# mingfeisun/DeepMimic_mujoco

Hardware: AMD Instinct MI355X
Metric: env-steps/sec (higher is better)
Workload: dtype f64

## Files before the change

deepmimic_mujoco_amd/csrc/slot_kernel.h:

```cpp
#pragma once

#include <cstddef>

#include "env_kernel.h"

namespace dm {

constexpr int SLOTS = 4, SW = 16;
#ifndef DM_SLOT_MAXROWS
#define DM_SLOT_MAXROWS 40
#endif
constexpr int SLOT_MAXROWS = DM_SLOT_MAXROWS, SLOT_MAXLIMROWS = 16, SLOT_MAXCON = 13, SLOT_MAXFRAME = 8, SLOT_MAXCAND = 32, SLOT_BOXSLOTS = 3;
constexpr int SLOT_EXTROWS = SLOT_MAXROWS - 2 * SW;
static_assert(SLOT_EXTROWS == 8 || SLOT_EXTROWS == 0, "the partial third row set holds eight rows (or is absent)");
constexpr int PAIR_PASSES = MAXPAIR / SW;
static_assert(MAXPAIR <= 128 && NG <= 16, "a candidate word holds the pair number in 7 bits and both geom numbers in 4 bits each");
constexpr int DOF_PASSES = (NV + SW - 1) / SW, HINGE_PASSES = (NU + SW - 1) / SW, Q_PASSES = (NQ + SW - 1) / SW, ENT_PASSES = (310 + SW - 1) / SW;

#ifndef DM_SLOT_ASSUME
#define DM_SLOT_ASSUME 31
#endif
#define DM_SLOT_LANE_AT(bit, x) (((DM_SLOT_ASSUME) >> (bit)) & 1 ? dmw::launder_slot_lane(x) : dmw::launder(x))

template <class R>
// ... 639 lines not shown
    }
    SlotSolveLTStep<I - 1, NVEC, R>::run(x, qLD, nxt);
  }
};
template <int NVEC, class R> struct SlotSolveLTStep<0, NVEC, R> { static DM_DEV void run(R (*)[NV], const R*, const R*) {} };
template <int NVEC, class R> DM_DEV void slot_solve_LT(R (*x)[NV], const R* qLD) {
  R cur[14];
  dmw::reload_fence();
  load_factor_row<NV - 1>(cur, qLD);
  SlotSolveLTStep<NV - 1, NVEC, R>::run(x, qLD, cur);
}

template <int D, class R>
DM_DEV void slot_load_dof_operands(R* dst, const SlotShared<R>& s) {
  if constexpr (D < NV) {
#pragma unroll
    for (int r = 0; r < 6; r++) dst[r] = s.cdof[D][r];
    dst[6] = s.qvel[D]; dst[7] = s.qws[D];
  }
}
template <int D, int NS, class R>
struct SlotRowStep {
  static DM_DEV void run(R (*y)[NV], RowAcc<R>* ra, const SlotShared<R>& s, const R* cur) {
    R nxt[8];
    dmw::reload_fence();
    slot_load_dof_operands<D + 1>(nxt, s);
    dmw::sched_fence();
#pragma unroll
    for (int k = 0; k < NS; k++) {
      const int pb = (int)(D < 32 ? (ra[k].plus_lo >> D) & 1u : (ra[k].plus_hi >> (D - 32)) & 1u);
      const int mb = (int)(D < 32 ? (ra[k].minus_lo >> D) & 1u : (ra[k].minus_hi >> (D - 32)) & 1u);
      R j = ra[k].w[0] * cur[0] + ra[k].w[1] * cur[1] + ra[k].w[2] * cur[2] + ra[k].w[3] * cur[3] + ra[k].w[4] * cur[4] + ra[k].w[5] * cur[5];
      j = (j + ra[k].w7) * (R)(pb - mb);
      ra[k].vel += j * cur[6]; ra[k].jws += j * cur[7];
      y[k][D] = j;
      dmw::pin_value(ra[k].vel); dmw::pin_value(ra[k].jws);
    }
    SlotRowStep<D + 1, NS, R>::run(y, ra, s, nxt);
  }
};
template <int NS, class R> struct SlotRowStep<NV, NS, R> { static DM_DEV void run(R (*)[NV], RowAcc<R>*, const SlotShared<R>&, const R*) {} };

template <int CC, int NS, class R>
DM_DEV void slot_acol(R (*AR)[16 * NS], const R (*y)[NV]) {
#pragma unroll
  for (int k = 0; k < NS; k++) {
    R acc0 = 0, acc1 = 0;
#pragma unroll
    for (int d = 0; d + 8 <= NV; d += 8) dmw::row_fmac8<CC % 16>(acc0, acc1, &y[CC / 16][d], &y[k][d]);
#pragma unroll
    for (int d = NV / 8 * 8; d < NV; d += 2) { dmw::row_fmac_old<CC % 16>(acc0, y[CC / 16][d], y[k][d]); dmw::row_fmac_old<CC % 16>(acc1, y[CC / 16][d + 1], y[k][d + 1]); }
    AR[k][CC] = acc0 + acc1;
  }
}
template <int C, int NS, class R>
struct SlotACols {
  static DM_DEV void run(R (*AR)[16 * NS], const R (*y)[NV], int nmax) {
    if constexpr (C < 16 * NS) {
      slot_acol<C, NS, R>(AR, y); slot_acol<C + 1, NS, R>(AR, y); slot_acol<C + 2, NS, R>(AR, y); slot_acol<C + 3, NS, R>(AR, y);
      if (C + 4 < nmax) SlotACols<C + 4, NS, R>::run(AR, y, nmax);
    }
  }
};
template <int CC, int NS, class R>
DM_DEV void slot_warm_col(R (*AR)[16 * NS], R* t, const R* f, const R* ndinv) {
#pragma unroll
  for (int k = 0; k < NS; k++) { AR[k][CC] *= ndinv[k]; dmw::row_fmac_old<CC % 16>(t[k], f[CC / 16], AR[k][CC]); }
}
template <int C, int NS, class R>
struct SlotWarm {
  static DM_DEV void run(R (*AR)[16 * NS], R* t, const R* f, const R* ndinv, int nmax) {
    if constexpr (C < 16 * NS) {
      slot_warm_col<C, NS, R>(AR, t, f, ndinv); slot_warm_col<C + 1, NS, R>(AR, t, f, ndinv); slot_warm_col<C + 2, NS, R>(AR, t, f, ndinv); slot_warm_col<C + 3, NS, R>(AR, t, f, ndinv);
      if (C + 4 < nmax) SlotWarm<C + 4, NS, R>::run(AR, t, f, ndinv, nmax);
    }
  }
};
template <int CC, int NS, class R>
DM_DEV void slot_sweep_rows4(const R (*AR)[16 * NS], R* t, R* tsave, const R* nf0, const R* oh) {
  static_assert(CC % 4 == 0, "row groups of four");
  if constexpr (NS == 1) dmw::pgs_rows4<CC % 16>(t[0], tsave[0], nf0[0], &AR[0][CC], &oh[CC % 16]);
  else dmw::pgs_rows4_2<CC % 16>(t[CC / 16], tsave[CC / 16], t[1 - CC / 16], nf0[CC / 16], &AR[CC / 16][CC], &AR[1 - CC / 16][CC], &oh[CC % 16]);
}
template <int C, int NS, class R>
struct SlotSweep {
  static DM_DEV void run(const R (*AR)[16 * NS], R* t, R* tsave, const R* nf0, const R* oh, int nmax) {
    if constexpr (C < 16 * NS) {
      slot_sweep_rows4<C, NS, R>(AR, t, tsave, nf0, oh);
      if (C + 4 < nmax) SlotSweep<C + 4, NS, R>::run(AR, t, tsave, nf0, oh, nmax);
    }
  }
};
template <int CC, class R>
DM_DEV void slot_assemble_row(R* ws, const R (*fy)[NV], R one) {
#pragma unroll
  for (int d = 0; d + 8 <= NV; d += 8) dmw::row_add8<CC % 16>(&ws[d], &fy[CC / 16][d], one);
#pragma unroll
  for (int d = NV / 8 * 8; d < NV; d++) dmw::row_fmac_old<CC % 16>(ws[d], fy[CC / 16][d], one);
}
template <int C, int NS, class R>
struct SlotAssemble {
  static DM_DEV void run(R* ws, const R (*fy)[NV], R one, int nmax) {
    if constexpr (C < 16 * NS) {
      slot_assemble_row<C, R>(ws, fy, one); slot_assemble_row<C + 1, R>(ws, fy, one); slot_assemble_row<C + 2, R>(ws, fy, one); slot_assemble_row<C + 3, R>(ws, fy, one);
      if (C + 4 < nmax) SlotAssemble<C + 4, NS, R>::run(ws, fy, one, nmax);
    }
  }
};

template <class R>
DM_DEV R row_reduce8(const R* p, int sl) {
  const bool b3 = (sl & 8) != 0, b2 = (sl & 4) != 0, b1 = (sl & 2) != 0;
  R q[4], r2[2];
#pragma unroll
  for (int i = 0; i < 4; i++) { const R keep = b3 ? p[4 + i] : p[i], send = b3 ? p[i] : p[4 + i]; q[i] = keep + dmw::perm_row_mirror(send); }
#pragma unroll
  for (int i = 0; i < 2; i++) { const R keep = b2 ? q[2 + i] : q[i], send = b2 ? q[i] : q[2 + i]; r2[i] = keep + dmw::perm_half_mirror(send); }
  const R keep = b1 ? r2[1] : r2[0], send = b1 ? r2[0] : r2[1];
  R v = keep + dmw::perm_xor2(send);
  v += dmw::perm_xor1(v);
  return v;
}
template <int J, class R>
DM_DEV void slot_ext_col(R (*U)[SLOT_EXTROWS], R* B, const R (*y)[NV], const R* y3) {
#pragma unroll
  for (int k = 0; k < 3; k++) {
    const R* mine = k < 2 ? y[k] : y3;
    R acc0 = 0, acc1 = 0;
#pragma unroll
    for (int d = 0; d + 8 <= NV; d += 8) dmw::row_fmac8<2 * J>(acc0, acc1, &y3[d], &mine[d]);
#pragma unroll
    for (int d = NV / 8 * 8; d < NV; d += 2) { dmw::row_fmac_old<2 * J>(acc0, y3[d], mine[d]); dmw::row_fmac_old<2 * J>(acc1, y3[d + 1], mine[d + 1]); }
    if (k < 2) U[k][J] = acc0 + acc1; else B[J] = acc0 + acc1;
  }
}
template <int J, class R>
struct SlotExtCols {
  static DM_DEV void run(R (*U)[SLOT_EXTROWS], R* B, const R (*y)[NV], const R* y3, int next) {
    if constexpr (J < SLOT_EXTROWS) {
      slot_ext_col<J, R>(U, B, y, y3); slot_ext_col<J + 1, R>(U, B, y, y3); slot_ext_col<J + 2, R>(U, B, y, y3); slot_ext_col<J + 3, R>(U, B, y, y3);
      if (J + 4 < next) SlotExtCols<J + 4, R>::run(U, B, y, y3, next);
    }
  }
};
template <int J, class R>
struct SlotExtWarm {
  static DM_DEV void run(R (*U)[SLOT_EXTROWS], R* B, R* t, R f3, const R* ndinv, R ndinv3, int next) {
    if constexpr (J < SLOT_EXTROWS) {
#pragma unroll
      for (int j = J; j < J + 4; j++) { U[0][j] *= ndinv[0]; U[1][j] *= ndinv[1]; B[j] *= ndinv3; }
      dmw::row_fmac_old<2 * J>(t[0], f3, U[0][J]); dmw::row_fmac_old<2 * J>(t[1], f3, U[1][J]);
      dmw::row_fmac_old<2 * J + 2>(t[0], f3, U[0][J + 1]); dmw::row_fmac_old<2 * J + 2>(t[1], f3, U[1][J + 1]);
      dmw::row_fmac_old<2 * J + 4>(t[0], f3, U[0][J + 2]); dmw::row_fmac_old<2 * J + 4>(t[1], f3, U[1][J + 2]);
      dmw::row_fmac_old<2 * J + 6>(t[0], f3, U[0][J + 3]); dmw::row_fmac_old<2 * J + 6>(t[1], f3, U[1][J + 3]);
      if (J + 4 < next) SlotExtWarm<J + 4, R>::run(U, B, t, f3, ndinv, ndinv3, next);
    }
  }
};
template <class R>
DM_DEV R slot_ext_residual(const R (*U)[SLOT_EXTROWS], const R* B, const R* f, const R* diag, R f3, R tb3, R ndinv3, int sl) {
  const R g0 = -(diag[0] * f[0]), g1 = -(diag[1] * f[1]);
  R p[SLOT_EXTROWS > 0 ? SLOT_EXTROWS : 1];
#pragma unroll
  for (int j = 0; j < SLOT_EXTROWS; j++) p[j] = U[0][j] * g0 + U[1][j] * g1;
  R t3 = tb3 + ndinv3 * row_reduce8(p, sl);
  dmw::dpp_settle();
  dmw::row_fmac_old<0>(t3, f3, B[0]); dmw::row_fmac_old<2>(t3, f3, B[1]); dmw::row_fmac_old<4>(t3, f3, B[2]); dmw::row_fmac_old<6>(t3, f3, B[3]);
  dmw::row_fmac_old<8>(t3, f3, B[4]); dmw::row_fmac_old<10>(t3, f3, B[5]); dmw::row_fmac_old<12>(t3, f3, B[6]); dmw::row_fmac_old<14>(t3, f3, B[7]);
  return t3;
}
template <int J, class R>
struct SlotExtSweep {
  static DM_DEV void run(const R (*U)[SLOT_EXTROWS], const R* B, R& t3, R& tsave3, R* t, R nf03, const R* oh, int next) {
    if constexpr (J < SLOT_EXTROWS) {
      dmw::pgs_row3<2 * J>(t3, tsave3, t[0], t[1], nf03, B[J], U[0][J], U[1][J], oh[2 * J]);
// ... 194 lines not shown
  R AR[NF][NC];
#pragma unroll
  for (int k = 0; k < NF; k++)
#pragma unroll
    for (int c = 0; c < NC; c++) { AR[k][c] = 0; dmw::pin_value(AR[k][c]); }
  dmw::dpp_settle();
  SlotACols<0, NF, R>::run(AR, y, nmax);
  R diag[NF];
#pragma unroll
  for (int k = 0; k < NF; k++) {
    R dg = 1;
#pragma unroll
    for (int c = 0; c < 16; c++) { if (sl == c) { AR[k][16 * k + c] += active[k] ? Rr[k] : R(0); dg = AR[k][16 * k + c]; } }
    diag[k] = active[k] ? dg : R(1);
  }
  SLOT_STAMP(10)
  typedef decltype(dmw::park(R(0))) ParkedR;
  ParkedR ypark[NF == 2 ? NF : 1][NF == 2 ? NV : 1];
  if constexpr (NF == 2) {
    if constexpr (!EXT) {
      if (sl == 0) {
#pragma unroll
        for (int d = 0; d < NV; d++) s.tau[d] = y[NF][d];
      }
    }
#pragma unroll
    for (int k = 0; k < NF; k++)
#pragma unroll
      for (int d = 0; d < NV; d++) ypark[k][d] = dmw::park(y[k][d]);
#pragma unroll
    for (int k = 0; k < NF; k++)
#pragma unroll
      for (int c = 0; c < NC; c++) dmw::pin_value(AR[k][c]);
    if constexpr (EXT) {
#pragma unroll
      for (int j = 0; j < NX; j++) { dmw::pin_value(U[0][j]); dmw::pin_value(U[1][j]); dmw::pin_value(B3[j]); }
    }
  }
  R ndinv[NF], tb[NF], t[NF];
#pragma unroll
  for (int k = 0; k < NF; k++) { ndinv[k] = active[k] ? R(-1) / diag[k] : R(0); dmw::pin_value(ndinv[k]); tb[k] = bb[k] * ndinv[k]; t[k] = tb[k]; }
  SlotWarm<0, NF, R>::run(AR, t, f, ndinv, nmax);
  R ndinv3 = 0, tb3 = 0;
  if constexpr (EXT) {
    ndinv3 = active3 ? R(-1) / diag3 : R(0); dmw::pin_value(ndinv3);
    tb3 = bb3 * ndinv3;
    dmw::dpp_settle();
    SlotExtWarm<0, R>::run(U, B3, t, f3, ndinv, ndinv3, nmax - 2 * SW);
  }
  {
    R c = 0;
#pragma unroll
    for (int k = 0; k < NF; k++) { const R res = -t[k] * diag[k]; c += active[k] ? f[k] * (R(0.5) * (res - bb[k]) + bb[k]) : R(0); }
    if constexpr (EXT) {
      const R t3 = slot_ext_residual(U, B3, f, diag, f3, tb3, ndinv3, sl);
      const R res = -t3 * diag3;
      c += active3 ? f3 * (R(0.5) * (res - bb3) + bb3) : R(0);
    }
    const R cost = dmw::sum16(c);
    if (cost > 0) {
#pragma unroll
      for (int k = 0; k < NF; k++) { f[k] = 0; t[k] = tb[k]; }
      f3 = 0;
    }
  }
  SLOT_STAMP(11)
  const int maxiter = dmw::uniform(M.iterations);
  R pgs_scale = M.pgs_scale, pgs_tol = M.tolerance, pgs_detect = M.pgs_detect;
  dmw::pin_value(pgs_scale); dmw::pin_value(pgs_tol); dmw::pin_value(pgs_detect);
  int iter = 0;
  bool frozen = nefc == 0 || maxiter <= 0, anybad = false;
  if (frozen) {
#pragma unroll
    for (int k = 0; k < NF; k++) t[k] = 0;
  }
  R oh[16];
#pragma unroll
  for (int i = 0; i < 16; i++) { oh[i] = sl == i ? R(1) : R(0); dmw::pin_value(oh[i]); }
  R nf[NF], nf3 = -f3;
#pragma unroll
  for (int k = 0; k < NF; k++) nf[k] = -f[k];
  R pgs_ntol = -pgs_tol;
  dmw::pin_value(pgs_ntol);
  auto sweep = [&](R& chg, bool& bad) {
    const int nm = dmw::launder_uniform(nmax);
    R tsave[NF];
#pragma unroll
    for (int k = 0; k < NF; k++) tsave[k] = 0;
    SlotSweep<0, NF, R>::run(AR, t, tsave, nf, oh, nm);
    bad = false;
#pragma unroll
    for (int k = 0; k < NF; k++) {
      const R delta = dmw::max_raw(nf[k], tsave[k]);
      const R change = (delta * diag[k]) * (R(0.5) * delta - tsave[k]);
      chg = k == 0 ? change : chg + change;
      nf[k] -= delta; bad = bad || (change > pgs_detect);
    }
    if constexpr (EXT) {
      R fnow[NF];
#pragma unroll
      for (int k = 0; k < NF; k++) fnow[k] = -nf[k];
      const R f3now = -nf3;
      R t3 = slot_ext_residual(U, B3, fnow, diag, f3now, tb3, ndinv3, sl);
      t3 = frozen ? R(0) : t3;
      R tsave3 = 0;
      SlotExtSweep<0, R>::run(U, B3, t3, tsave3, t, nf3, oh, nm - 2 * SW);
      const R delta = dmw::max_raw(nf3, tsave3);
      const R change = (delta * diag3) * (R(0.5) * delta - tsave3);
      nf3 -= delta; chg += change; bad = bad || (change > pgs_detect);
    }
  };
  if (dmw::ballot(!frozen) != 0ull) {
    R chg; bool bad;
    sweep(chg, bad);
    if (!frozen) { iter = 1; anybad = bad; }
    bool more = true;
    while (more) {
      R nfprev[NF], nfprev3 = nf3;
#pragma unroll
      for (int k = 0; k < NF; k++) nfprev[k] = nf[k];
      const R schg = dmw::sum16(chg) * pgs_scale;
      R chg2; bool bad2;
      sweep(chg2, bad2);
      const bool act = !frozen;
      const bool conv = (int)act & ((int)(schg > pgs_ntol) | (int)(iter >= maxiter));
#pragma unroll
      for (int k = 0; k < NF; k++) {
        nf[k] = conv ? nfprev[k] : nf[k];
        t[k] = conv ? R(0) : t[k];
      }
      if constexpr (EXT) nf3 = conv ? nfprev3 : nf3;
      const bool go = (int)act & (int)!conv;
      iter += go ? 1 : 0;
      anybad = (int)anybad | ((int)go & (int)bad2);
      frozen = (int)frozen | (int)conv;
      chg = chg2;
      more = dmw::ballot(!frozen) != 0ull;
      if (PROF) prof[6] += 1;
    }
  }
#pragma unroll
  for (int k = 0; k < NF; k++) f[k] = -nf[k];
  f3 = -nf3;
  if (PROF && NS >= 2) { prof[22] += dmw::clk() - pt0; }
  if (PROF && NS == 3) { prof[27] += dmw::clk() - pt0; }
  SLOT_STAMP(12)
  if (PROF) { prof[14] += nmax; prof[15] += 1; }
  if (dmw::row_ballot(anybad, lane) != 0u) ovf |= 16 | 64;
  if (dbg) {
#pragma unroll
    for (int k = 0; k < NF; k++) if (active[k]) {
      double* o = dbg->out + (34 * 34 + 34 * 3 + 42 + 3) + (sl + 16 * k) * (34 + 6) + 34;
      o[0] = (double)pos[k]; o[1] = (double)margin[k]; o[2] = (double)Rr[k]; o[3] = (double)aref[k]; o[4] = (double)bb[k]; o[5] = (double)f[k];
    }
  }
  R fy3[EXT ? NV : 1];
  if constexpr (EXT) {
    const R* y3lds = &s.qd.o.qacc[0];
    const R f3a = active3 ? f3 : R(0);
#pragma unroll
    for (int d = 0; d < NV; d++) { fy3[d] = ((sl & 1) == 0 ? y3lds[d * SLOT_EXTROWS + (sl >> 1)] : R(0)) * f3a; dmw::pin_value(fy3[d]); }
  }
  if constexpr (NF == 2) {
    dmw::sync();
#pragma unroll
    for (int d = 0; d < NV; d++) y[NF][d] = s.tau[d];
  }
#pragma unroll
  for (int k = 0; k < NF; k++) {
    const R fk = active[k] ? f[k] : R(0);
#pragma unroll
    for (int d = 0; d < NV; d++) { if constexpr (NF == 2) y[k][d] = dmw::unpark(ypark[k][d]); y[k][d] *= fk; dmw::pin_value(y[k][d]); }
  }
  R ws[NV];
#pragma unroll
  for (int d = 0; d < NV; d++) { ws[d] = 0; dmw::pin_value(ws[d]); }
  R one = 1;
  dmw::pin_value(one);
  dmw::dpp_settle();
  SlotAssemble<0, NF, R>::run(ws, y, one, nmax);
  if constexpr (EXT) SlotExtAssemble<0, R>::run(ws, fy3, one, nmax - 2 * SW);
#pragma unroll
  for (int d = 0; d < NV; d++) ws[d] = (ws[d] + y[NF][d]) * s.dsq[d];
  solve_L(ws, s.r2.qLD);
  if (sl == 0) {
#pragma unroll
    for (int d = 0; d < NV; d++) s.qd.o.qacc[d] = ws[d];
    s.solver_iter = iter;
  }
  dmw::sync();
  SLOT_STAMP(13)
  if (PROF && NS >= 2) prof[24] += dmw::clk() - pt_enter;
  if (PROF && NS == 3) prof[26] += dmw::clk() - pt_enter;
#undef SLOT_STAMP
}

#if !defined(DM_WAVE_TESTBENCH)
template <class R, int MAXR>
static __device__ __noinline__ int slot_rows_call(const DevModel<R>* M, SlotShared<R>* s, int sl, int lane, int* ovf) {
  int o = *ovf;
  const int n = slot_rows<R, false, MAXR>(*dmw::in_constant(M), *dmw::in_lds(s), sl, lane, o, (long long*)0);
  *ovf = o;
  return n;
}
#endif

template <class R>
DM_DEV void slot_smooth_solve(SlotShared<R>& s, int sl, const DebugOut* dbg) {
  R x[1][NV];
#pragma unroll
  for (int d = 0; d < NV; d++) x[0][d] = s.tau[d];
  slot_solve_LT<1>(x, s.r2.qLD);
#pragma unroll
  for (int d = 0; d < NV; d++) { x[0][d] *= s.dsq[d]; dmw::pin_value(x[0][d]); }
#pragma unroll
  for (int d = 0; d < NV; d++) x[0][d] = (R(0) + x[0][d]) * s.dsq[d];
  solve_L(x[0], s.r2.qLD);
  if (sl == 0) {
#pragma unroll
    for (int d = 0; d < NV; d++) { s.qd.o.qacc[d] = x[0][d]; if (dbg) dbg->out[34 * 34 + 34 + d] = (double)x[0][d]; }
    s.solver_iter = 0;
  }
// ... 57 lines not shown
```

deepmimic_mujoco_amd/csrc/wave.h:

```cpp
#pragma once

#if defined(DM_WAVE_TESTBENCH)
#include "wave_testbench.h"
#else
#include <hip/hip_runtime.h>

#define DM_DEV __device__ __forceinline__
#define DM_DEV_NOINLINE __device__ __noinline__
#ifndef DM_NO_STATIC_CALLS
#define DM_STATIC_CALLS 1
#define DM_DEV_CALL64 static __device__ __noinline__
#else
#define DM_DEV_CALL64 __device__ __noinline__
#endif
#define DM_CONSTANT __device__ constexpr

namespace dmw {
DM_DEV int lane() { return (int)(threadIdx.x & 63u); }
DM_DEV void sync() { __builtin_amdgcn_fence(__ATOMIC_SEQ_CST, "wavefront"); __builtin_amdgcn_wave_barrier(); }
DM_DEV void sync_mem() { __syncthreads(); }
DM_DEV unsigned long long ballot(bool p) { return __ballot(p); }
DM_DEV int shfl_i(int v, int src) { return __shfl(v, src, 64); }
DM_DEV double shfl(double v, int src) { return __shfl(v, src, 64); }
DM_DEV float shfl(float v, int src) { return __shfl(v, src, 64); }
DM_DEV double shfl_xor(double v, int m) { return __shfl_xor(v, m, 64); }
DM_DEV float shfl_xor(float v, int m) { return __shfl_xor(v, m, 64); }
DM_DEV int shfl_xor_i(int v, int m) { return __shfl_xor(v, m, 64); }
DM_DEV int shfl_up_i(int v, int d) { return __shfl_up(v, d, 64); }
DM_DEV double bcast(double v, int src) {
  int lo = __double2loint(v), hi = __double2hiint(v);
  lo = __builtin_amdgcn_readlane(lo, src);
  hi = __builtin_amdgcn_readlane(hi, src);
  return __hiloint2double(hi, lo);
}
DM_DEV float bcast(float v, int src) { return __int_as_float(__builtin_amdgcn_readlane(__float_as_int(v), src)); }
DM_DEV int bcast_i(int v, int src) { return __builtin_amdgcn_readlane(v, src); }
template <int CTRL>
DM_DEV double dpp_f64(double v) {
  int lo = __double2loint(v), hi = __double2hiint(v);
  lo = __builtin_amdgcn_update_dpp(0, lo, CTRL, 0xf, 0xf, true);
  hi = __builtin_amdgcn_update_dpp(0, hi, CTRL, 0xf, 0xf, true);
  return __hiloint2double(hi, lo);
}
template <int CTRL>
DM_DEV float dpp_f32(float v) { return __int_as_float(__builtin_amdgcn_update_dpp(0, __float_as_int(v), CTRL, 0xf, 0xf, true)); }
DM_DEV float perm_xor1(float v) { return dpp_f32<0xB1>(v); }
DM_DEV float perm_xor2(float v) { return dpp_f32<0x4E>(v); }
DM_DEV float perm_half_mirror(float v) { return dpp_f32<0x141>(v); }
DM_DEV float perm_row_mirror(float v) { return dpp_f32<0x140>(v); }
DM_DEV double perm_xor1(double v) { return dpp_f64<0xB1>(v); }
DM_DEV double perm_xor2(double v) { return dpp_f64<0x4E>(v); }
DM_DEV double perm_half_mirror(double v) { return dpp_f64<0x141>(v); }
DM_DEV double perm_row_mirror(double v) { return dpp_f64<0x140>(v); }
DM_DEV int uniform(int v) { return __builtin_amdgcn_readfirstlane(v); }
DM_DEV bool uniform(bool v) { return __builtin_amdgcn_readfirstlane((int)v) != 0; }
DM_DEV double rcp_fast(double x) {
  double r = __builtin_amdgcn_rcp(x);
  double e = __builtin_fma(-x, r, 1.0); r = __builtin_fma(e, r, r);
  e = __builtin_fma(-x, r, 1.0); r = __builtin_fma(e, r, r);
  return r;
}
DM_DEV float rcp_fast(float x) { return 1.0f / x; }
DM_DEV void mfma_16x16x4(double a, double b, double (&d)[4]) {
  typedef double v4d __attribute__((ext_vector_type(4)));
  v4d c = {d[0], d[1], d[2], d[3]};
  c = __builtin_amdgcn_mfma_f64_16x16x4f64(a, b, c, 0, 0, 0);
  d[0] = c[0]; d[1] = c[1]; d[2] = c[2]; d[3] = c[3];
}
DM_DEV void mfma_16x16x4(float a, float b, float (&d)[4]) {
  typedef float v4f __attribute__((ext_vector_type(4)));
  v4f c = {d[0], d[1], d[2], d[3]};
  c = __builtin_amdgcn_mfma_f32_16x16x4f32(a, b, c, 0, 0, 0);
  d[0] = c[0]; d[1] = c[1]; d[2] = c[2]; d[3] = c[3];
}
DM_DEV int mfma_row(int lane_id, int v, double) { return (lane_id >> 4) + 4 * v; }
DM_DEV int mfma_row(int lane_id, int v, float) { return 4 * (lane_id >> 4) + v; }
DM_DEV double max_raw(double a, double b) { double r; asm("v_max_f64 %0, %1, %2" : "=v"(r) : "v"(a), "v"(b)); return r; }
DM_DEV float max_raw(float a, float b) { float r; asm("v_max_f32 %0, %1, %2" : "=v"(r) : "v"(a), "v"(b)); return r; }
DM_DEV long long clk() { return (long long)__builtin_readcyclecounter(); }
DM_DEV void sched_fence() { __builtin_amdgcn_sched_barrier(0); }
DM_DEV int pin_zero() { int z = 0; asm volatile("" : "+s"(z)); return z; }
DM_DEV void pin_value(double& v) { asm volatile("" : "+v"(v)); }
DM_DEV void pin_value(float& v) { asm volatile("" : "+v"(v)); }
DM_DEV int launder(int v) { asm volatile("" : "+v"(v)); return v; }
DM_DEV int launder_slot_lane(int v) { asm volatile("" : "+v"(v)); __builtin_assume(v >= 0 && v < 16); return v; }
DM_DEV unsigned long long launder(unsigned long long v) { asm volatile("" : "+v"(v)); return v; }
DM_DEV int launder_uniform(int v) { asm volatile("" : "+s"(v)); return v; }
template <class T> DM_DEV T* uniform_ptr(T* p) {
  const unsigned long long v = (unsigned long long)p;
  const unsigned lo = __builtin_amdgcn_readfirstlane((unsigned)v), hi = __builtin_amdgcn_readfirstlane((unsigned)(v >> 32));
  return (T*)(((unsigned long long)hi << 32) | lo);
}
template <class T> DM_DEV T* in_lds(T* p) {
#if defined(__HIP_DEVICE_COMPILE__)
  __builtin_assume(__builtin_amdgcn_is_shared((const void*)p));
#endif
  return p;
}
template <class T> DM_DEV T* in_global(T* p) {
  __attribute__((address_space(1))) T* g = (__attribute__((address_space(1))) T*)uniform_ptr(p);
  asm volatile("" : "+s"(g));
  return (T*)g;
}
template <class T> DM_DEV const T* in_constant(const T* p) {
// ... 10 lines not shown
  x = __builtin_amdgcn_update_dpp(0ll, x, 0x150 + I, 0xf, 0xf, true);
  return __longlong_as_double(x);
}
template <int I> DM_DEV float row_bcast(float v) { return __int_as_float(__builtin_amdgcn_update_dpp(0, __float_as_int(v), 0x150 + I, 0xf, 0xf, true)); }
template <int I> DM_DEV int row_bcast_i(int v) { return __builtin_amdgcn_update_dpp(0, v, 0x150 + I, 0xf, 0xf, true); }
template <int I> DM_DEV void row_fmac(double& acc, double x, double y) {
  asm volatile("s_nop 1\n\tv_fmac_f64_dpp %0, %1, %2 row_newbcast:%3 row_mask:0xf bank_mask:0xf" : "+v"(acc) : "v"(x), "v"(y), "n"(I));
}
template <int I> DM_DEV void row_fmac(float& acc, float x, float y) { acc += row_bcast<I>(x) * y; }
template <int I> DM_DEV void row_fmac_old(double& acc, double x, double y) {
  asm volatile("s_nop 1\n\tv_fmac_f64_dpp %0, %1, %2 row_newbcast:%3 row_mask:0xf bank_mask:0xf" : "+v"(acc) : "v"(x), "v"(y), "n"(I));
}
template <int I> DM_DEV void row_fmac_old(float& acc, float x, float y) { acc += row_bcast<I>(x) * y; }
#define DM_FMAC_DPP(acc, x, y) "v_fmac_f64_dpp " acc ", " x ", " y " row_newbcast:%18 row_mask:0xf bank_mask:0xf\n\t"
template <int I> DM_DEV void row_fmac8(double& acc0, double& acc1, const double* x, const double* y) {
  asm volatile("s_nop 1\n\t" DM_FMAC_DPP("%0", "%2", "%10") DM_FMAC_DPP("%1", "%3", "%11") DM_FMAC_DPP("%0", "%4", "%12") DM_FMAC_DPP("%1", "%5", "%13")
               DM_FMAC_DPP("%0", "%6", "%14") DM_FMAC_DPP("%1", "%7", "%15") DM_FMAC_DPP("%0", "%8", "%16") DM_FMAC_DPP("%1", "%9", "%17")
               : "+v"(acc0), "+v"(acc1)
               : "v"(x[0]), "v"(x[1]), "v"(x[2]), "v"(x[3]), "v"(x[4]), "v"(x[5]), "v"(x[6]), "v"(x[7]),
                 "v"(y[0]), "v"(y[1]), "v"(y[2]), "v"(y[3]), "v"(y[4]), "v"(y[5]), "v"(y[6]), "v"(y[7]), "n"(I));
}
#undef DM_FMAC_DPP
#define DM_FMAC_DPP(acc, x) "v_fmac_f64_dpp " acc ", " x ", %16 row_newbcast:%17 row_mask:0xf bank_mask:0xf\n\t"
template <int I> DM_DEV void row_add8(double* a, const double* x, double one) {
  asm volatile("s_nop 1\n\t" DM_FMAC_DPP("%0", "%8") DM_FMAC_DPP("%1", "%9") DM_FMAC_DPP("%2", "%10") DM_FMAC_DPP("%3", "%11")
               DM_FMAC_DPP("%4", "%12") DM_FMAC_DPP("%5", "%13") DM_FMAC_DPP("%6", "%14") DM_FMAC_DPP("%7", "%15")
               : "+v"(a[0]), "+v"(a[1]), "+v"(a[2]), "+v"(a[3]), "+v"(a[4]), "+v"(a[5]), "+v"(a[6]), "+v"(a[7])
               : "v"(x[0]), "v"(x[1]), "v"(x[2]), "v"(x[3]), "v"(x[4]), "v"(x[5]), "v"(x[6]), "v"(x[7]), "v"(one), "n"(I));
}
#undef DM_FMAC_DPP
template <int I> DM_DEV void row_fmac8(float& acc0, float& acc1, const float* x, const float* y) { for (int k = 0; k < 8; k++) { if (k & 1) acc1 += row_bcast<I>(x[k]) * y[k]; else acc0 += row_bcast<I>(x[k]) * y[k]; } }
template <int I> DM_DEV void row_add8(float* a, const float* x, float one) { for (int k = 0; k < 8; k++) a[k] += row_bcast<I>(x[k]) * one; }
template <int I> DM_DEV void pgs_row(double& t, double& tsave, double nf0, double a, double onehot) {
  double delta;
  asm volatile("v_max_f64 %0, %3, %1\n\tv_fma_f64 %2, %5, %1, %2\n\ts_nop 0\n\tv_fmac_f64_dpp %1, %0, %4 row_newbcast:%6 row_mask:0xf bank_mask:0xf"
               : "=&v"(delta), "+v"(t), "+v"(tsave) : "v"(nf0), "v"(a), "v"(onehot), "n"(I));
}
template <int I> DM_DEV void pgs_row2(double& t_own, double& tsave_own, double& t_other, double nf0, double a_own, double a_other, double onehot) {
  double delta;
  asm volatile("v_max_f64 %0, %4, %1\n\tv_fma_f64 %2, %7, %1, %2\n\ts_nop 0\n\tv_fmac_f64_dpp %1, %0, %5 row_newbcast:%8 row_mask:0xf bank_mask:0xf\n\t"
               "v_fmac_f64_dpp %3, %0, %6 row_newbcast:%8 row_mask:0xf bank_mask:0xf"
               : "=&v"(delta), "+v"(t_own), "+v"(tsave_own), "+v"(t_other) : "v"(nf0), "v"(a_own), "v"(a_other), "v"(onehot), "n"(I));
}
template <int I> DM_DEV void pgs_row3(double& t3, double& tsave3, double& t0, double& t1, double nf0, double b, double u0, double u1, double onehot) {
  double delta;
  asm volatile("v_max_f64 %0, %5, %1\n\tv_fma_f64 %2, %9, %1, %2\n\ts_nop 0\n\tv_fmac_f64_dpp %1, %0, %6 row_newbcast:%10 row_mask:0xf bank_mask:0xf\n\t"
               "v_fmac_f64_dpp %3, %0, %7 row_newbcast:%10 row_mask:0xf bank_mask:0xf\n\tv_fmac_f64_dpp %4, %0, %8 row_newbcast:%10 row_mask:0xf bank_mask:0xf"
               : "=&v"(delta), "+v"(t3), "+v"(tsave3), "+v"(t0), "+v"(t1) : "v"(nf0), "v"(b), "v"(u0), "v"(u1), "v"(onehot), "n"(I));
}
template <int I> DM_DEV void pgs_row3(float& t3, float& tsave3, float& t0, float& t1, float nf0, float b, float u0, float u1, float onehot) {
  const float d = max_raw(nf0, t3); tsave3 += onehot * t3; const float bc = row_bcast<I>(d); t3 += bc * b; t0 += bc * u0; t1 += bc * u1;
}
#define DM_PGS1(D, A, OH, I) "v_max_f64 " D ", %3, %0\n\tv_fma_f64 %1, " OH ", %0, %1\n\ts_nop 0\n\tv_fmac_f64_dpp %0, " D ", " A " row_newbcast:" I " row_mask:0xf bank_mask:0xf\n\t"
template <int I0> DM_DEV void pgs_rows4(double& t, double& tsave, double nf0, const double* a, const double* oh) {
  double d;
  asm volatile(DM_PGS1("%2", "%4", "%8", "%12") DM_PGS1("%2", "%5", "%9", "%13") DM_PGS1("%2", "%6", "%10", "%14") DM_PGS1("%2", "%7", "%11", "%15")
               : "+v"(t), "+v"(tsave), "=&v"(d)
               : "v"(nf0), "v"(a[0]), "v"(a[1]), "v"(a[2]), "v"(a[3]), "v"(oh[0]), "v"(oh[1]), "v"(oh[2]), "v"(oh[3]), "n"(I0), "n"(I0 + 1), "n"(I0 + 2), "n"(I0 + 3));
}
#undef DM_PGS1
template <int I0> DM_DEV void pgs_rows4_2(double& t_own, double& tsave_own, double& t_other, double nf0, const double* a_own, const double* a_other, const double* oh) {
  double d0, d1;
  asm volatile(
      "v_max_f64 %3, %5, %0\n\tv_fma_f64 %1, %14, %0, %1\n\ts_nop 0\n\tv_fmac_f64_dpp %0, %3, %6 row_newbcast:%18 row_mask:0xf bank_mask:0xf\n\t"
      "v_max_f64 %4, %5, %0\n\tv_fma_f64 %1, %15, %0, %1\n\tv_fmac_f64_dpp %2, %3, %10 row_newbcast:%18 row_mask:0xf bank_mask:0xf\n\tv_fmac_f64_dpp %0, %4, %7 row_newbcast:%19 row_mask:0xf bank_mask:0xf\n\t"
      "v_max_f64 %3, %5, %0\n\tv_fma_f64 %1, %16, %0, %1\n\tv_fmac_f64_dpp %2, %4, %11 row_newbcast:%19 row_mask:0xf bank_mask:0xf\n\tv_fmac_f64_dpp %0, %3, %8 row_newbcast:%20 row_mask:0xf bank_mask:0xf\n\t"
      "v_max_f64 %4, %5, %0\n\tv_fma_f64 %1, %17, %0, %1\n\tv_fmac_f64_dpp %2, %3, %12 row_newbcast:%20 row_mask:0xf bank_mask:0xf\n\tv_fmac_f64_dpp %0, %4, %9 row_newbcast:%21 row_mask:0xf bank_mask:0xf\n\t"
      "s_nop 0\n\tv_fmac_f64_dpp %2, %4, %13 row_newbcast:%21 row_mask:0xf bank_mask:0xf"
      : "+v"(t_own), "+v"(tsave_own), "+v"(t_other), "=&v"(d0), "=&v"(d1)
      : "v"(nf0), "v"(a_own[0]), "v"(a_own[1]), "v"(a_own[2]), "v"(a_own[3]), "v"(a_other[0]), "v"(a_other[1]), "v"(a_other[2]), "v"(a_other[3]),
        "v"(oh[0]), "v"(oh[1]), "v"(oh[2]), "v"(oh[3]), "n"(I0), "n"(I0 + 1), "n"(I0 + 2), "n"(I0 + 3));
}
template <int I> DM_DEV void pgs_row(float& t, float& tsave, float nf0, float a, float onehot) { const float d = max_raw(nf0, t); tsave += onehot * t; t += row_bcast<I>(d) * a; }
template <int I> DM_DEV void pgs_row2(float& t_own, float& tsave_own, float& t_other, float nf0, float a_own, float a_other, float onehot) {
  const float d = max_raw(nf0, t_own); tsave_own += onehot * t_own; const float b = row_bcast<I>(d); t_own += b * a_own; t_other += b * a_other;
}
template <int I0> DM_DEV void pgs_rows4(float& t, float& tsave, float nf0, const float* a, const float* oh) {
  pgs_row<I0>(t, tsave, nf0, a[0], oh[0]); pgs_row<I0 + 1>(t, tsave, nf0, a[1], oh[1]); pgs_row<I0 + 2>(t, tsave, nf0, a[2], oh[2]); pgs_row<I0 + 3>(t, tsave, nf0, a[3], oh[3]);
}
template <int I0> DM_DEV void pgs_rows4_2(float& t_own, float& tsave_own, float& t_other, float nf0, const float* a_own, const float* a_other, const float* oh) {
  pgs_row2<I0>(t_own, tsave_own, t_other, nf0, a_own[0], a_other[0], oh[0]); pgs_row2<I0 + 1>(t_own, tsave_own, t_other, nf0, a_own[1], a_other[1], oh[1]);
  pgs_row2<I0 + 2>(t_own, tsave_own, t_other, nf0, a_own[2], a_other[2], oh[2]); pgs_row2<I0 + 3>(t_own, tsave_own, t_other, nf0, a_own[3], a_other[3], oh[3]);
}
DM_DEV void dpp_settle() { asm volatile("s_nop 4"); }
struct Parked { int lo, hi; };
DM_DEV Parked park(double v) {
  Parked p;
  asm volatile("v_accvgpr_write_b32 %0, %2\n\tv_accvgpr_write_b32 %1, %3" : "=a"(p.lo), "=a"(p.hi) : "v"(__double2loint(v)), "v"(__double2hiint(v)));
  return p;
}
DM_DEV double unpark(const Parked& p) {
  int lo, hi;
  asm volatile("v_accvgpr_read_b32 %0, %2\n\tv_accvgpr_read_b32 %1, %3" : "=v"(lo), "=v"(hi) : "a"(p.lo), "a"(p.hi));
  return __hiloint2double(hi, lo);
}
struct ParkedF { int x; };
DM_DEV ParkedF park(float v) { ParkedF p; asm volatile("v_accvgpr_write_b32 %0, %1" : "=a"(p.x) : "v"(__float_as_int(v))); return p; }
DM_DEV float unpark(const ParkedF& p) { int x; asm volatile("v_accvgpr_read_b32 %0, %1" : "=v"(x) : "a"(p.x)); return __int_as_float(x); }
DM_DEV int global_counter_next(int* p) { return atomicAdd(p, 1); }
DM_DEV unsigned row_ballot(bool p, int lane_id) { return (unsigned)((__ballot(p) >> (lane_id & 48)) & 0xffffull); }
}
#endif

namespace dmw {
DM_DEV double sum8(double v) { v += perm_xor1(v); v += perm_xor2(v); v += perm_half_mirror(v); return v; }
DM_DEV double sum16(double v) { v = sum8(v); v += perm_row_mirror(v); return v; }
DM_DEV double wave_sum(double v) {
  v = sum16(v);
  return ((bcast(v, 0) + bcast(v, 16)) + bcast(v, 32)) + bcast(v, 48);
}
#if !defined(DM_WAVE_TESTBENCH)
DM_DEV float sum8(float v) { v += perm_xor1(v); v += perm_xor2(v); v += perm_half_mirror(v); return v; }
DM_DEV float sum16(float v) { v = sum8(v); v += perm_row_mirror(v); return v; }
DM_DEV float wave_sum(float v) {
  v = sum16(v);
  return ((bcast(v, 0) + bcast(v, 16)) + bcast(v, 32)) + bcast(v, 48);
}
#endif
DM_DEV int wave_exclusive_scan(int v, int lane_id, int* total) {
  const unsigned long long below = (1ull << lane_id) - 1ull;
  int pre = 0, tot = 0;
#pragma unroll
  for (int b = 0; b < 5; b++) {
    const unsigned long long m = ballot(((v >> b) & 1) != 0);
    pre += __builtin_popcountll(m & below) << b;
    tot += __builtin_popcountll(m) << b;
  }
  *total = tot;
  return pre;
}
}
```

Measured before the change: 20.71 million.

## Overlap PGS convergence reduction with the next sweep's row updates

Interleaves the 16-lane cost-change reduction (DPP stages) into the inline-asm row updates of the following PGS sweep, so the reduction no longer sits serially between sweeps. Loop control is restructured around a trip counter and a cheaper ballot builtin, and the cost change is computed with explicit FMA and non-contracted ops to keep rounding identical. The asm hardcodes v250-v253, which constrains register allocation and could cause spills. It also adds coupling between sweep length and reduction stage count.

New measurement: 20.70 million. No clear change (-0.0%).

```diff
diff --git a/deepmimic_mujoco_amd/csrc/slot_kernel.h b/deepmimic_mujoco_amd/csrc/slot_kernel.h
--- a/deepmimic_mujoco_amd/csrc/slot_kernel.h
+++ b/deepmimic_mujoco_amd/csrc/slot_kernel.h
@@ -745,15 +745,33 @@
   if constexpr (NS == 1) dmw::pgs_rows4<CC % 16>(t[0], tsave[0], nf0[0], &AR[0][CC], &oh[CC % 16]);
   else dmw::pgs_rows4_2<CC % 16>(t[CC / 16], tsave[CC / 16], t[1 - CC / 16], nf0[CC / 16], &AR[CC / 16][CC], &AR[1 - CC / 16][CC], &oh[CC % 16]);
 }
-template <int C, int NS, class R>
+template <int CC, int NS, class R>
+DM_DEV void slot_sweep_rows4_red(const R (*AR)[16 * NS], R* t, R* tsave, const R* nf0, const R* oh, R& red) {
+  static_assert(CC % 4 == 0 && CC < (NS == 1 ? 8 : 16), "row groups of four; four stages");
+  if constexpr (NS == 1) dmw::pgs_rows4_red2<CC, CC / 2>(t[0], tsave[0], nf0[0], &AR[0][CC], &oh[CC], red);
+  else dmw::pgs_rows4_2_red<CC, CC / 4>(t[0], tsave[0], t[1], nf0[0], &AR[0][CC], &AR[1][CC], &oh[CC], red);
+}
+template <int C, int NS, bool RED, class R>
 struct SlotSweep {
-  static DM_DEV void run(const R (*AR)[16 * NS], R* t, R* tsave, const R* nf0, const R* oh, int nmax) {
+  static DM_DEV void run(const R (*AR)[16 * NS], R* t, R* tsave, const R* nf0, const R* oh, int nmax, R& red, R scale) {
     if constexpr (C < 16 * NS) {
-      slot_sweep_rows4<C, NS, R>(AR, t, tsave, nf0, oh);
-      if (C + 4 < nmax) SlotSweep<C + 4, NS, R>::run(AR, t, tsave, nf0, oh, nmax);
+      if constexpr (RED && C < (NS == 1 ? 8 : 16)) slot_sweep_rows4_red<C, NS, R>(AR, t, tsave, nf0, oh, red);
+      else {
+        if constexpr (RED && C == 16) red = dmw::mul_rn(red, scale);
+        slot_sweep_rows4<C, NS, R>(AR, t, tsave, nf0, oh);
+      }
+      if constexpr (C + 4 < 16 * NS) { if (C + 4 < nmax) SlotSweep<C + 4, NS, RED, R>::run(AR, t, tsave, nf0, oh, nmax, red, scale); }
     }
   }
 };
+template <int NS, bool RED, class R>
+DM_DEV void slot_sweep(const R (*AR)[16 * NS], R* t, R* tsave, const R* nf0, const R* oh, int nmax, R& red, R scale) {
+  SlotSweep<0, NS, RED, R>::run(AR, t, tsave, nf0, oh, nmax, red, scale);
+  if constexpr (RED && NS == 1) {
+    if (nmax <= 4) { dmw::dpp_settle(); red = dmw::sum16_stage<3>(dmw::sum16_stage<2>(red)); }
+    red = dmw::mul_rn(red, scale);
+  }
+}
 template <int CC, class R>
 DM_DEV void slot_assemble_row(R* ws, const R (*fy)[NV], R one) {
 #pragma unroll
@@ -1114,19 +1132,23 @@
   for (int k = 0; k < NF; k++) nf[k] = -f[k];
   R pgs_ntol = -pgs_tol;
   dmw::pin_value(pgs_ntol);
-  auto sweep = [&](R& chg, bool& bad) {
+  auto sweep = [&](auto redtag, R& red, R& chg, bool& bad) {
+    constexpr bool RED = decltype(redtag)::value;
     const int nm = dmw::launder_uniform(nmax);
     R tsave[NF];
 #pragma unroll
     for (int k = 0; k < NF; k++) tsave[k] = 0;
-    SlotSweep<0, NF, R>::run(AR, t, tsave, nf, oh, nm);
+    slot_sweep<NF, RED, R>(AR, t, tsave, nf, oh, nm, red, pgs_scale);
     bad = false;
+    static_assert(NF <= 2, "the cost change below is written for one or two row sets");
+    R p0 = 0, q0 = 0;
 #pragma unroll
     for (int k = 0; k < NF; k++) {
       const R delta = dmw::max_raw(nf[k], tsave[k]);
-      const R change = (delta * diag[k]) * (R(0.5) * delta - tsave[k]);
-      chg = k == 0 ? change : chg + change;
-      nf[k] -= delta; bad = bad || (change > pgs_detect);
+      const R p = dmw::mul_rn(delta, diag[k]), q = dmw::mul_sub(R(0.5), delta, tsave[k]);
+      const R change = dmw::mul_rn(p, q);
+      if (k == 0) { chg = change; p0 = p; q0 = q; } else chg = dmw::mul_add(p0, q0, change);
+      nf[k] = dmw::sub_rn(nf[k], delta); bad = bad || (change > pgs_detect);
     }
     if constexpr (EXT) {
       R fnow[NF];
@@ -1143,33 +1165,37 @@
     }
   };
   if (dmw::ballot(!frozen) != 0ull) {
-    R chg; bool bad;
-    sweep(chg, bad);
-    if (!frozen) { iter = 1; anybad = bad; }
+    R chg, none = 0; bool bad;
+    sweep(std::false_type(), none, chg, bad);
+    if (!frozen) anybad = bad;
+    int trip = 1;
+    bool act = !frozen;
+    iter = act ? 0 : -1;
     bool more = true;
     while (more) {
       R nfprev[NF], nfprev3 = nf3;
 #pragma unroll
       for (int k = 0; k < NF; k++) nfprev[k] = nf[k];
-      const R schg = dmw::sum16(chg) * pgs_scale;
+      R schg = chg;
       R chg2; bool bad2;
-      sweep(chg2, bad2);
-      const bool act = !frozen;
-      const bool conv = (int)act & ((int)(schg > pgs_ntol) | (int)(iter >= maxiter));
+      sweep(std::true_type(), schg, chg2, bad2);
+      const bool capped = trip >= maxiter;
+      const bool conv = (int)act & ((int)(schg > pgs_ntol) | (int)capped);
 #pragma unroll
       for (int k = 0; k < NF; k++) {
         nf[k] = conv ? nfprev[k] : nf[k];
         t[k] = conv ? R(0) : t[k];
       }
-      if constexpr (EXT) nf3 = conv ? nfprev3 : nf3;
-      const bool go = (int)act & (int)!conv;
-      iter += go ? 1 : 0;
-      anybad = (int)anybad | ((int)go & (int)bad2);
-      frozen = (int)frozen | (int)conv;
+      if constexpr (EXT) { nf3 = conv ? nfprev3 : nf3; frozen = (int)frozen | (int)conv; }
+      iter = conv ? trip : iter;
+      act = iter == 0;
+      anybad = (int)anybad | ((int)act & (int)bad2);
       chg = chg2;
-      more = dmw::ballot(!frozen) != 0ull;
+      trip++;
+      more = dmw::lane_mask(act) != 0ull;
       if (PROF) prof[6] += 1;
     }
+    iter = iter < 0 ? 0 : iter;
   }
 #pragma unroll
   for (int k = 0; k < NF; k++) f[k] = -nf[k];
diff --git a/deepmimic_mujoco_amd/csrc/wave.h b/deepmimic_mujoco_amd/csrc/wave.h
--- a/deepmimic_mujoco_amd/csrc/wave.h
+++ b/deepmimic_mujoco_amd/csrc/wave.h
@@ -2,6 +2,19 @@
 
 #if defined(DM_WAVE_TESTBENCH)
 #include "wave_testbench.h"
+namespace dmw {
+inline unsigned long long lane_mask(bool pr) { return ballot(pr); }
+template <int S> inline double sum16_stage(double v) {
+  static_assert(S >= 0 && S < 4, "sum16 has four stages");
+  if constexpr (S == 0) return v + perm_xor1(v); else if constexpr (S == 1) return v + perm_xor2(v); else if constexpr (S == 2) return v + perm_half_mirror(v); else return v + perm_row_mirror(v);
+}
+template <int I0, int S, class T> inline void pgs_rows4_red2(T& t, T& tsave, T nf0, const T* a, const T* oh, T& acc) { pgs_rows4<I0>(t, tsave, nf0, a, oh); acc = sum16_stage<S + 1>(sum16_stage<S>(acc)); }
+template <int I0, int S, class T> inline void pgs_rows4_2_red(T& t_own, T& tsave_own, T& t_other, T nf0, const T* a_own, const T* a_other, const T* oh, T& acc) {
+  pgs_rows4_2<I0>(t_own, tsave_own, t_other, nf0, a_own, a_other, oh); acc = sum16_stage<S>(acc);
+}
+template <class T> inline T mul_sub(T a, T b, T c) { return a * b - c; }
+template <class T> inline T mul_add(T a, T b, T c) { return a * b + c; }
+}
 #else
 #include <hip/hip_runtime.h>
 
@@ -20,6 +33,7 @@
 DM_DEV void sync() { __builtin_amdgcn_fence(__ATOMIC_SEQ_CST, "wavefront"); __builtin_amdgcn_wave_barrier(); }
 DM_DEV void sync_mem() { __syncthreads(); }
 DM_DEV unsigned long long ballot(bool p) { return __ballot(p); }
+DM_DEV unsigned long long lane_mask(bool p) { return __builtin_amdgcn_ballot_w64(p); }
 DM_DEV int shfl_i(int v, int src) { return __shfl(v, src, 64); }
 DM_DEV double shfl(double v, int src) { return __shfl(v, src, 64); }
 DM_DEV float shfl(float v, int src) { return __shfl(v, src, 64); }
@@ -196,6 +210,60 @@
   pgs_row2<I0>(t_own, tsave_own, t_other, nf0, a_own[0], a_other[0], oh[0]); pgs_row2<I0 + 1>(t_own, tsave_own, t_other, nf0, a_own[1], a_other[1], oh[1]);
   pgs_row2<I0 + 2>(t_own, tsave_own, t_other, nf0, a_own[2], a_other[2], oh[2]); pgs_row2<I0 + 3>(t_own, tsave_own, t_other, nf0, a_own[3], a_other[3], oh[3]);
 }
+template <int S> DM_DEV double sum16_stage(double v) {
+  static_assert(S >= 0 && S < 4, "sum16 has four stages");
+  if constexpr (S == 0) return v + perm_xor1(v); else if constexpr (S == 1) return v + perm_xor2(v); else if constexpr (S == 2) return v + perm_half_mirror(v); else return v + perm_row_mirror(v);
+}
+template <int S> DM_DEV float sum16_stage(float v) {
+  static_assert(S >= 0 && S < 4, "sum16 has four stages");
+  if constexpr (S == 0) return v + perm_xor1(v); else if constexpr (S == 1) return v + perm_xor2(v); else if constexpr (S == 2) return v + perm_half_mirror(v); else return v + perm_row_mirror(v);
+}
+#define DM_RIDE_LO(CTRL) "v_mov_b32_dpp v252, v250 " CTRL " row_mask:0xf bank_mask:0xf bound_ctrl:1"
+#define DM_RIDE_HI(CTRL) "v_mov_b32_dpp v253, v251 " CTRL " row_mask:0xf bank_mask:0xf bound_ctrl:1"
+#define DM_RIDE_ADD "v_add_f64 v[250:251], v[250:251], v[252:253]"
+#define DM_PGS1R(A, OH, I, SLOT) "v_max_f64 %[d], %[nf0], %[t]\n\tv_fma_f64 %[ts], %[" OH "], %[t], %[ts]\n\t" SLOT "\n\tv_fmac_f64_dpp %[t], %[d], %[" A "] row_newbcast:%[" I "] row_mask:0xf bank_mask:0xf\n\t"
+#define DM_PGS_ROWS4_RED2(CA, CB)                                                                                                                                \
+  asm volatile(DM_PGS1R("a0", "oh0", "i0", DM_RIDE_LO(CA)) DM_PGS1R("a1", "oh1", "i1", DM_RIDE_HI(CA)) DM_PGS1R("a2", "oh2", "i2", DM_RIDE_ADD)                   \
+               DM_PGS1R("a3", "oh3", "i3", DM_RIDE_LO(CB) "\n\t" DM_RIDE_HI(CB)) DM_RIDE_ADD                                                                      \
+               : [t] "+v"(t), [ts] "+v"(tsave), [d] "=&v"(d), "+{v[250:251]}"(acc), "=&{v[252:253]}"(tmp)                                                         \
+               : [nf0] "v"(nf0), [a0] "v"(a[0]), [a1] "v"(a[1]), [a2] "v"(a[2]), [a3] "v"(a[3]), [oh0] "v"(oh[0]), [oh1] "v"(oh[1]), [oh2] "v"(oh[2]), [oh3] "v"(oh[3]), \
+                 [i0] "n"(I0), [i1] "n"(I0 + 1), [i2] "n"(I0 + 2), [i3] "n"(I0 + 3))
+template <int I0, int S> DM_DEV void pgs_rows4_red2(double& t, double& tsave, double nf0, const double* a, const double* oh, double& acc) {
+  static_assert(S == 0 || S == 2, "stages 0, 1 or stages 2, 3");
+  double d, tmp;
+  if constexpr (S == 0) DM_PGS_ROWS4_RED2("quad_perm:[1,0,3,2]", "quad_perm:[2,3,0,1]"); else DM_PGS_ROWS4_RED2("row_half_mirror", "row_mirror");
+}
+#undef DM_PGS_ROWS4_RED2
+#undef DM_PGS1R
+#define DM_PGS_ROWS4_2_RED(CTRL)                                                                                                                                 \
+  asm volatile(                                                                                                                                                  \
+      "v_max_f64 %[d0], %[nf0], %[t]\n\tv_fma_f64 %[ts], %[oh0], %[t], %[ts]\n\t" DM_RIDE_LO(CTRL) "\n\tv_fmac_f64_dpp %[t], %[d0], %[a0] row_newbcast:%[i0] row_mask:0xf bank_mask:0xf\n\t" \
+      "v_max_f64 %[d1], %[nf0], %[t]\n\tv_fma_f64 %[ts], %[oh1], %[t], %[ts]\n\t" DM_RIDE_HI(CTRL) "\n\tv_fmac_f64_dpp %[u], %[d0], %[b0] row_newbcast:%[i0] row_mask:0xf bank_mask:0xf\n\tv_fmac_f64_dpp %[t], %[d1], %[a1] row_newbcast:%[i1] row_mask:0xf bank_mask:0xf\n\t" \
+      "v_max_f64 %[d0], %[nf0], %[t]\n\tv_fma_f64 %[ts], %[oh2], %[t], %[ts]\n\tv_fmac_f64_dpp %[u], %[d1], %[b1] row_newbcast:%[i1] row_mask:0xf bank_mask:0xf\n\tv_fmac_f64_dpp %[t], %[d0], %[a2] row_newbcast:%[i2] row_mask:0xf bank_mask:0xf\n\t" \
+      "v_max_f64 %[d1], %[nf0], %[t]\n\tv_fma_f64 %[ts], %[oh3], %[t], %[ts]\n\tv_fmac_f64_dpp %[u], %[d0], %[b2] row_newbcast:%[i2] row_mask:0xf bank_mask:0xf\n\tv_fmac_f64_dpp %[t], %[d1], %[a3] row_newbcast:%[i3] row_mask:0xf bank_mask:0xf\n\t" \
+      DM_RIDE_ADD "\n\tv_fmac_f64_dpp %[u], %[d1], %[b3] row_newbcast:%[i3] row_mask:0xf bank_mask:0xf"                                                           \
+      : [t] "+v"(t_own), [ts] "+v"(tsave_own), [u] "+v"(t_other), [d0] "=&v"(d0), [d1] "=&v"(d1), "+{v[250:251]}"(acc), "=&{v[252:253]}"(tmp)                     \
+      : [nf0] "v"(nf0), [a0] "v"(a_own[0]), [a1] "v"(a_own[1]), [a2] "v"(a_own[2]), [a3] "v"(a_own[3]), [b0] "v"(a_other[0]), [b1] "v"(a_other[1]),              \
+        [b2] "v"(a_other[2]), [b3] "v"(a_other[3]), [oh0] "v"(oh[0]), [oh1] "v"(oh[1]), [oh2] "v"(oh[2]), [oh3] "v"(oh[3]),                                      \
+        [i0] "n"(I0), [i1] "n"(I0 + 1), [i2] "n"(I0 + 2), [i3] "n"(I0 + 3))
+template <int I0, int S> DM_DEV void pgs_rows4_2_red(double& t_own, double& tsave_own, double& t_other, double nf0, const double* a_own, const double* a_other, const double* oh, double& acc) {
+  static_assert(S >= 0 && S < 4, "sum16 has four stages");
+  double d0, d1, tmp;
+  if constexpr (S == 0) DM_PGS_ROWS4_2_RED("quad_perm:[1,0,3,2]"); else if constexpr (S == 1) DM_PGS_ROWS4_2_RED("quad_perm:[2,3,0,1]");
+  else if constexpr (S == 2) DM_PGS_ROWS4_2_RED("row_half_mirror"); else DM_PGS_ROWS4_2_RED("row_mirror");
+}
+#undef DM_PGS_ROWS4_2_RED
+#undef DM_RIDE_LO
+#undef DM_RIDE_HI
+#undef DM_RIDE_ADD
+template <int I0, int S> DM_DEV void pgs_rows4_red2(float& t, float& tsave, float nf0, const float* a, const float* oh, float& acc) { pgs_rows4<I0>(t, tsave, nf0, a, oh); acc = sum16_stage<S + 1>(sum16_stage<S>(acc)); }
+template <int I0, int S> DM_DEV void pgs_rows4_2_red(float& t_own, float& tsave_own, float& t_other, float nf0, const float* a_own, const float* a_other, const float* oh, float& acc) {
+  pgs_rows4_2<I0>(t_own, tsave_own, t_other, nf0, a_own, a_other, oh); acc = sum16_stage<S>(acc);
+}
+DM_DEV double mul_sub(double a, double b, double c) { return __builtin_fma(a, b, -c); }
+DM_DEV float mul_sub(float a, float b, float c) { return __builtin_fmaf(a, b, -c); }
+DM_DEV double mul_add(double a, double b, double c) { return __builtin_fma(a, b, c); }
+DM_DEV float mul_add(float a, float b, float c) { return __builtin_fmaf(a, b, c); }
 DM_DEV void dpp_settle() { asm volatile("s_nop 4"); }
 struct Parked { int lo, hi; };
 DM_DEV Parked park(double v) {
@@ -231,6 +299,18 @@
   return ((bcast(v, 0) + bcast(v, 16)) + bcast(v, 32)) + bcast(v, 48);
 }
 #endif
+template <class T> DM_DEV T mul_rn(T a, T b) {
+#if defined(__clang__)
+#pragma clang fp contract(off)
+#endif
+  return a * b;
+}
+template <class T> DM_DEV T sub_rn(T a, T b) {
+#if defined(__clang__)
+#pragma clang fp contract(off)
+#endif
+  return a - b;
+}
 DM_DEV int wave_exclusive_scan(int v, int lane_id, int* total) {
   const unsigned long long below = (1ull << lane_id) - 1ull;
   int pre = 0, tot = 0;
```
